# hanruihua/RDA-planner

Hardware: AMD Instinct MI355X
Metric: MPC steps/sec (ADMM early stop or iter_num cap: see residuals), T=20, N_obs=200 (higher is better)
Workload: dtype f64; 1 GPU; north-star: acker rectangle robot, T=20, N_obs=200 static seeded polygons, E=4, iter_num=4, iter_threshold=0.2, ro1=200; parallelism=single GPU

## Files before the change

rda_planner_amd/csrc/lammuz_device.h:

```cpp
#pragma once
#include <hip/hip_runtime.h>
#include <math.h>

#pragma clang fp contract(on)

namespace lmz {

constexpr int EMAX = 8;
constexpr int RMAX = 8;
constexpr double SIGN_TOL = 1e-12;

struct WaveLDS {
    double A[EMAX][2];
    double b[EMAX];
    double q[EMAX];
    double M[EMAX][2];
    unsigned char lamc[40];
    double vtx[28][2];
    int npv, nlv;
};
struct RobotLDS {
    double G[RMAX][2];
    double h[RMAX];
    unsigned char muc[40]; int nmv;
// ... 370 lines not shown
            Sol s;
            if (eval_candidate(W, Rb, P, il, im, ic, s)) {
                s.id = 2 * (il * nm + im) + ic;
                if (s.cost < best.cost || (s.cost == best.cost && s.id < best.id)) best = s;
            }
            mark(1 + 2 * ic + (itn < 1 ? itn : 1)); ++itn;
        }
        double bc = best.cost; int bid = best.id;
#pragma unroll
        for (int off = 32; off >= 1; off >>= 1) {
            double oc = __shfl_xor(bc, off, 64); int oid = __shfl_xor(bid, off, 64);
            if (oc < bc || (oc == bc && oid < bid)) { bc = oc; bid = oid; }
        }
        unsigned long long win = __ballot(best.id == bid);
        int src = __ffsll((long long)win) - 1;
        best.cost = __shfl(best.cost, src, 64); best.id = bid;
        best.m = __shfl(best.m, src, 64); best.H0 = __shfl(best.H0, src, 64); best.H1 = __shfl(best.H1, src, 64);
        best.i1 = __shfl(best.i1, src, 64); best.i2 = __shfl(best.i2, src, 64);
        best.j1 = __shfl(best.j1, src, 64); best.j2 = __shfl(best.j2, src, 64);
        best.l1 = __shfl(best.l1, src, 64); best.l2 = __shfl(best.l2, src, 64);
        best.g1 = __shfl(best.g1, src, 64); best.g2 = __shfl(best.g2, src, 64);
        mark(5 + ic);
        if (best.m >= 0) break;
        if (ic == 0) best.cost += 0.5 * best.m * best.m;
    }
}

template <int CTRL> __device__ __forceinline__ double dpp_mov_f64(double v)
{
    int lo = __builtin_amdgcn_update_dpp(0, __double2loint(v), CTRL, 0xf, 0xf, false);
    int hi = __builtin_amdgcn_update_dpp(0, __double2hiint(v), CTRL, 0xf, 0xf, false);
    return __hiloint2double(hi, lo);
}
__device__ __forceinline__ double wave_max(double v)
{
    double o;
    o = dpp_mov_f64<0xB1>(v); v = o > v ? o : v;
    o = dpp_mov_f64<0x4E>(v); v = o > v ? o : v;
    o = dpp_mov_f64<0x141>(v); v = o > v ? o : v;
    o = dpp_mov_f64<0x140>(v); v = o > v ? o : v;
    o = __shfl_xor(v, 16, 64); v = o > v ? o : v;
    o = __shfl_xor(v, 32, 64); v = o > v ? o : v;
    return v;
}

__device__ __forceinline__ double row_max(double v)
{
    double o;
    o = dpp_mov_f64<0xB1>(v); v = o > v ? o : v;
    o = dpp_mov_f64<0x4E>(v); v = o > v ? o : v;
    o = dpp_mov_f64<0x141>(v); v = o > v ? o : v;
    o = dpp_mov_f64<0x140>(v); v = o > v ? o : v;
    return v;
}
template <int GW> struct Grp {
    static __device__ __forceinline__ unsigned long long ballot(bool p, int lane)
    {
        const unsigned long long b = __ballot(p);
        if (GW == 64) return b;
        return (b >> (lane & 48)) & 0xffffull;
    }
    static __device__ __forceinline__ double max(double v) { return GW == 64 ? wave_max(v) : row_max(v); }
    template <typename Tv> static __device__ __forceinline__ Tv bcast(Tv v, int src) { return __shfl(v, src, GW); }
};

__device__ __forceinline__ int support_neighbour(int c, int n, const unsigned char *cand, int ncand, int k)
// ... 150 lines not shown
        const unsigned long long okb = Grp<GW>::ballot(ok, wlane);
        int src = -1;
        if ((okb & 1) && m0 >= 0) src = 0; else if ((okb & 2) && m1 < 0) src = 1;
        if (src >= 0) {
            take(s, src, 2 * (il * nm0 + im) + src);
            if (certify()) return true;
        }
    }
    if (GW >= 16) {
        const int q = (lane >> 1) & 7, c = lane & 1;
        int nil = -1, nim = -1;
        if (lane < 16) {
            if (q < 4) { nil = support_neighbour(il, E, W.lamc, W.nlv, q); nim = im; }
            else { nil = il; nim = support_neighbour(im, R, Rb.muc, Rb.nmv, q - 4); }
        }
        bool ok = false;
        if (lane < 16 && nil >= 0 && nim >= 0) ok = eval_candidate(W, Rb, P, nil, nim, c, s);
        const bool valid = ok && (c == 0 ? s.m >= 0 : s.m < 0);
        const unsigned long long vb = Grp<GW>::ballot(valid, wlane);
        const bool use = valid && !(c == 1 && ((vb >> (lane - 1)) & 1ull));
        const double cost = use ? s.cost : INFINITY;
        const double cmin = -Grp<GW>::max(-cost);
        if (cmin < INFINITY) {
            const unsigned long long wb = Grp<GW>::ballot(use && cost == cmin, wlane);
            const int src = __ffsll((long long)wb) - 1;
            const int cid = Grp<GW>::bcast(2 * (nil * nm0 + nim) + c, src);
            take(s, src, cid);
            if (certify()) return true;
        }
    }
    return false;
}

template <int GW> __device__ __forceinline__ bool central_normal_wave(const WaveLDS &W, const RobotLDS &Rb, const Params &P, int wlane, Sol &best)
{
    const int lane = wlane & (GW - 1);
    if (!(best.m > 0) || !(best.H0 * best.H0 + best.H1 * best.H1 < 1e-8)) return false;
    double as0 = 0, as1 = 0;
    if (P.norm2) { if (best.i1 >= 0) { as0 = best.l1; as1 = best.l2; } }
    else {
        if (best.i1 >= 0) { as0 += best.l1 * W.A[best.i1][0]; as1 += best.l1 * W.A[best.i1][1]; }
        if (best.i2 >= 0) { as0 += best.l2 * W.A[best.i2][0]; as1 += best.l2 * W.A[best.i2][1]; }
    }
    if (!(as0 * as0 + as1 * as1 >= 1.0 - 1e-9)) return false;
    const int nv = P.norm2 ? 1 : W.npv, nr = Rb.nrv;
    if (nr < 3 || (!P.norm2 && nv < 3) || nv * nr > 64 || nv > GW || nr > GW) return false;
    const double off = P.norm2 ? W.b[2] : 0.0;
    const double ins = rsqrt(as0 * as0 + as1 * as1), u0 = as0 * ins, u1 = as1 * ins;
    bool fail = false; double thi = INFINITY, tlo = INFINITY;
    for (int pi = lane; pi < nv * nr; pi += GW) {
        const int k = pi / nr, j = pi - k * nr;
        const double vx = P.norm2 ? W.b[0] : W.vtx[k][0], vy = P.norm2 ? W.b[1] : W.vtx[k][1];
        const double rx = Rb.rv[j][0], ry = Rb.rv[j][1];
        const double wx = P.px - vx + (P.cs * rx - P.sn * ry), wy = P.py - vy + (P.sn * rx + P.cs * ry);
        const double cj = P.xi0 * rx + P.xi1 * ry + P.kappa0 + off;
        const double n2 = wx * wx + wy * wy;
        if (!(n2 > 0)) fail = fail || cj < 0;
        else {
            const double inw = rsqrt(n2), q = -cj * inw, hx = wx * inw, hy = wy * inw;
            if (q >= 1.0) fail = true;
            else if (q > -1.0) {
                if (u0 * hx + u1 * hy < q - 1e-15) fail = true;
                else {
                    const double sb = sqrt((1.0 - q) * (1.0 + q));
                    const double epx = q * hx - sb * hy, epy = sb * hx + q * hy;
                    const double emx = q * hx + sb * hy, emy = -sb * hx + q * hy;
                    const double cp = u0 * epx + u1 * epy, sp = u0 * epy - u1 * epx;
                    const double cm = u0 * emx + u1 * emy, sm = emx * u1 - emy * u0;
                    double th = INFINITY, tl = INFINITY;
                    if (sp >= 0 && cp > -1.0) th = sp / (1.0 + cp);
                    else if (sp < 0 && sp > -1e-15) th = 0.0;
                    if (sm >= 0 && cm > -1.0) tl = sm / (1.0 + cm);
                    else if (sm < 0 && sm > -1e-15) tl = 0.0;
                    if (th < thi) thi = th;
                    if (tl < tlo) tlo = tl;
                }
            }
        }
    }
    if (Grp<GW>::ballot(fail, wlane)) return false;
    thi = -Grp<GW>::max(-thi); tlo = -Grp<GW>::max(-tlo);
    if (isinf(thi) && isinf(tlo)) return false;
    double chh, shh, chl, shl;
    if (isinf(thi)) { chh = 0; shh = 1; } else { const double r = rsqrt(1.0 + thi * thi); chh = r; shh = thi * r; }
    if (isinf(tlo)) { chl = 0; shl = 1; } else { const double r = rsqrt(1.0 + tlo * tlo); chl = r; shl = tlo * r; }
    const double Cr = chh * chl + shh * shl, Sr = shh * chl - chh * shl;
    const double a0 = u0 * Cr - u1 * Sr, a1 = u1 * Cr + u0 * Sr;
    int i1 = -1, i2 = -1; double l1 = 0, l2 = 0;
    if (P.norm2) { i1 = 0; i2 = 1; l1 = a0; l2 = a1; }
    else {
        const double val = lane < nv ? a0 * W.vtx[lane < nv ? lane : 0][0] + a1 * W.vtx[lane < nv ? lane : 0][1] : -INFINITY, mx = Grp<GW>::max(val);
        const int kb = __ffsll((long long)Grp<GW>::ballot(val == mx, wlane)) - 1;
        decode_pair((int)W.lamc[kb] - 1 - P.E, P.E, i1, i2);
        const double a00 = W.A[i1][0], a01 = W.A[i1][1], a10 = W.A[i2][0], a11 = W.A[i2][1], det = a00 * a11 - a01 * a10;
        l1 = (a0 * a11 - a10 * a1) / det;
        l2 = (a00 * a1 - a0 * a01) / det;
        if (l1 < -1e-9 || l2 < -1e-9) return false;
        if (l1 < 0) l1 = 0;
        if (l2 < 0) l2 = 0;
    }
    const double gx = -(P.cs * a0 + P.sn * a1) - P.xi0, gy = -(-P.sn * a0 + P.cs * a1) - P.xi1;
    int j1, j2; double g1, g2;
    {
        const double val = lane < nr ? gx * Rb.rv[lane < nr ? lane : 0][0] + gy * Rb.rv[lane < nr ? lane : 0][1] : -INFINITY, mx = Grp<GW>::max(val);
        const int jb = __ffsll((long long)Grp<GW>::ballot(val == mx, wlane)) - 1;
        decode_pair((int)Rb.muc[jb] - 1 - P.R, P.R, j1, j2);
        const double a00 = Rb.G[j1][0], a01 = Rb.G[j1][1], a10 = Rb.G[j2][0], a11 = Rb.G[j2][1], det = a00 * a11 - a01 * a10;
        g1 = (gx * a11 - a10 * gy) / det;
        g2 = (a00 * gy - gx * a01) / det;
        if (g1 < -1e-9 || g2 < -1e-9) return false;
        if (g1 < 0) g1 = 0;
        if (g2 < 0) g2 = 0;
    }
    double m = P.kappa0 - g1 * Rb.h[j1] - g2 * Rb.h[j2];
    double H0 = P.xi0 + g1 * Rb.G[j1][0] + g2 * Rb.G[j2][0], H1 = P.xi1 + g1 * Rb.G[j1][1] + g2 * Rb.G[j2][1];
    if (P.norm2) {
        m += l1 * W.q[0] + l2 * W.q[1] - W.q[2];
        H0 += l1 * W.M[0][0] + l2 * W.M[1][0] - W.M[2][0]; H1 += l1 * W.M[0][1] + l2 * W.M[1][1] - W.M[2][1];
    } else {
        m += l1 * W.q[i1] + l2 * W.q[i2];
        H0 += l1 * W.M[i1][0] + l2 * W.M[i2][0]; H1 += l1 * W.M[i1][1] + l2 * W.M[i2][1];
    }
    if (m < 0) return false;
    best.i1 = i1; best.i2 = i2; best.l1 = l1; best.l2 = l2; best.j1 = j1; best.j2 = j2; best.g1 = g1; best.g2 = g2;
    best.m = m; best.H0 = H0; best.H1 = H1;
    return true;
}

__device__ __forceinline__ double lam_of(const Sol &s, int norm2, int e)
{
    if (norm2) {
        if (s.i1 < 0) return 0.0;
        return e == 0 ? s.l1 : (e == 1 ? s.l2 : (e == 2 ? -hypot(s.l1, s.l2) : 0.0));
    }
    return e == s.i1 ? s.l1 : (e == s.i2 ? s.l2 : 0.0);
}
__device__ __forceinline__ double mu_of(const Sol &s, int j) { return j == s.j1 ? s.g1 : (j == s.j2 ? s.g2 : 0.0); }

}

#pragma clang fp contract(fast)
```

rda_planner_amd/csrc/rda_hip.hip:

```cpp
#include <hip/hip_runtime.h>
#include <climits>
#include <cstdio>
#include <cstdlib>
#include <cstring>
#include <vector>
#include <chrono>
#include <memory>
#include <dlfcn.h>
#include "../../include/rda_hip.h"
#include "host_buf.h"
#include "lammuz_device.h"
#include "lammuz_cp_device.h"
#include "lammuz_ip_device.h"
#include "su_device.h"
#include "scene_device.h"
#include "lidar_device.h"
#include "track_device.h"
#include "rollout_device.h"

#define HIPCHK(x) do { hipError_t e_ = (x); if (e_ != hipSuccess) { \
    fprintf(stderr, "librda_hip: %s failed: %s (%s:%d)\n", #x, hipGetErrorString(e_), __FILE__, __LINE__); return RDA_ERR_HIP; } } while (0)

struct Ctrl {
    int stop, iters, su_status, ipm_iters, st_tmp, it_tmp;
// ... 367 lines not shown
    return o;
}

__device__ __forceinline__ void block_partial(const Dev &d, int t, int j, const double (*rowv)[6], int q)
{
    const size_t bi = (size_t)t * d.J + j;
    if (q < NBS) {
        double acc = 0;
        for (int r = 0; r < GS; ++r) acc += rowv[r][q];
        __hip_atomic_store(bsum_arr(d, d.rank) + bi * NBS + q, acc, __ATOMIC_RELAXED, __HIP_MEMORY_SCOPE_AGENT);
    } else if (q == NBS) {
        unsigned long long m = 0;
        for (int r = 0; r < GS; ++r) m |= rowv[r][5] != 0.0 ? 1ull << r : 0ull;
        __hip_atomic_store(bmask_arr(d, d.rank) + bi, m, __ATOMIC_RELAXED, __HIP_MEMORY_SCOPE_AGENT);
    }
}
__device__ __forceinline__ void row_record(double *rv, const Dev &d, const RowOut &o, double px, double py)
{
    const su::RowTerm q = su::row_term(o.ax, o.ay, o.c4, o.c5, o.bl + o.c3, px, py, d.c.max_sd, true);
    rv[0] = q.aa; rv[1] = q.ga; rv[2] = q.gxa; rv[3] = o.res; rv[4] = o.hh; rv[5] = (!d.c.accelerated || q.near) ? 1.0 : 0.0;
}

__device__ __forceinline__ size_t hint_key(const Dev &d, int n, int t)
{
    int key = n;
    if (d.slot_src && n < d.src_used) { const int src = d.slot_src[n]; if (src >= 0 && src < d.src_cap) key = d.c.N + src; }
    return (size_t)t * d.hint_stride + key;
}
__device__ __forceinline__ int hint_read(const Dev &d, int par, int n, int t, bool first)
{
    return d.hint[(size_t)(par ^ 1) * d.hint_len + hint_key(d, n, first && t + 1 < d.c.T ? t + 1 : t)];
}
__device__ __forceinline__ void hint_write(const Dev &d, int par, int n, int t, int v) { d.hint[(size_t)par * d.hint_len + hint_key(d, n, t)] = v; }

__device__ __forceinline__ void lammuz_body(const Dev &d, const int block, const int it)
{
#pragma clang fp contract(on)
    __shared__ lmz::WaveLDS wl[4];
    __shared__ lmz::RobotLDS rb;
    const int T = d.c.T, N = d.c.N, E = d.c.E, R = d.c.R;
    if (d.ctrl->stop) return;
    const int lane = threadIdx.x & 63, wv = threadIdx.x >> 6;
    if (d.obstacle_num == 0) {
        if (block == 0 && d.rank == (N - 1) / d.Nloc)
            for (int t = threadIdx.x; t < T; t += 256) {
                int i = t * d.Nloc + (N - 1) % d.Nloc;
                coef_arr(d, d.rank, 0)[i] = 0; coef_arr(d, d.rank, 1)[i] = 0; coef_arr(d, d.rank, 2)[i] = 0;
                coef_arr(d, d.rank, 8)[i] = coef_arr(d, d.rank, 3)[i];
            }
        return;
    }
    if (threadIdx.x < 2 * R) rb.G[threadIdx.x >> 1][threadIdx.x & 1] = d.G[threadIdx.x];
    if (threadIdx.x >= 64 && threadIdx.x < 64 + R) rb.h[threadIdx.x - 64] = d.h[threadIdx.x - 64];
    if (threadIdx.x >= 128 && threadIdx.x < 128 + 40) rb.muc[threadIdx.x - 128] = d.muc[threadIdx.x - 128];
    if (threadIdx.x >= 192 && threadIdx.x < 192 + 56) (&rb.rv[0][0])[threadIdx.x - 192] = (&d.rv[0][0])[threadIdx.x - 192];
    if (threadIdx.x == 255) { rb.nmv = d.nmv; rb.nrv = d.nrv; }
    const int w = block * 4 + wv;
    int t, nl; unit_of(d, w, t, nl);
    const bool live = t < T && nl < d.Nlive;
    if (!live) { t = 0; nl = 0; }
    const int n = d.rank * d.Nloc + nl;
    lmz::WaveLDS &W = wl[wv];
    const size_t ao = ((size_t)n * d.nt + (d.nt > 1 ? t + 1 : 0)) * E;
    if (lane < 2 * E) W.A[lane >> 1][lane & 1] = d.A[ao * 2 + lane];
    if (lane < E) W.b[lane] = d.b[ao + lane];
    __syncthreads();
// ... 53 lines not shown
        res = (v - prev) * (v - prev); d.mu[o * R + j] = v;
    } else if (lane == E + R) {
        double old = d.z[zi];
        res = (znew - old) * (znew - old); d.z[zi] = znew;
    }
#pragma unroll
    for (int off = 32; off >= 1; off >>= 1) res += __shfl_xor(res, off, 64);
    if (lane == 0) {
        double ax = 0, ay = 0, bl = 0, mh = 0, gx = 0, gy = 0;
        for (int i = 0; i < E; ++i) {
            double v = lmz::lam_of(best, P.norm2, i);
            ax += v * W.A[i][0]; ay += v * W.A[i][1]; bl += v * W.b[i];
        }
        for (int j = 0; j < R; ++j) {
            double v = lmz::mu_of(best, j);
            mh += v * rb.h[j]; gx += v * rb.G[j][0]; gy += v * rb.G[j][1];
        }
        const double hx = gx + P.cs * ax + P.sn * ay, hy = gy - P.sn * ax + P.cs * ay;
        const double xin0 = P.xi0 + hx, xin1 = P.xi1 + hy;
        d.xi[2 * o] = xin0; d.xi[2 * o + 1] = xin1;
        const double im = ax * P.px + ay * P.py - bl - mh;
        const double zetan = zeta + im - dbar - znew;
        d.zeta[zi] = zetan;
        RowOut ro; ro.ax = ax; ro.ay = ay; ro.bl = bl; ro.c3 = mh + znew - zetan; ro.c4 = gx + xin0; ro.c5 = gy + xin1;
        ro.res = res; ro.hh = hx * hx + hy * hy;
        store_row(d, k, ro);
    }
}

__global__ __launch_bounds__(256) void k_lammuz(Dev d, int it) { lammuz_body(d, blockIdx.x, it); }

#ifdef RDA_LMZ_CLK
__device__ unsigned long long *g_lmz_clk = nullptr;
__device__ int *g_lmz_faillog = nullptr;
#endif
template <int MODE = 0, bool CW = false> __device__ __forceinline__ void lammuz_body_rows(const Dev &d, const int block, const int nblocks, const int it, const Fin &fin)
{
#pragma clang fp contract(on)
    constexpr int WPB = GS / 4;
    __shared__ lmz::WaveLDS wl[GS];
    __shared__ lmz::RobotLDS rb;
    __shared__ double rowv[MODE == 0 ? GS : 1][6];
    const int T = d.c.T, E = d.c.E, R = d.c.R;
#ifdef RDA_LMZ_CLK
    long long clk_prev = clock64(); const long long clk_in = clk_prev; bool clk_enum = false; const unsigned long long clk_wall_in = (unsigned long long)wall_clock64();
    unsigned long long *const clk_slot = g_lmz_clk ? g_lmz_clk + 16 * (size_t)(block * (GS / 4) + (threadIdx.x >> 6)) : nullptr;
#define LMZ_CLK(k) do { if (MODE == 0) { const long long now_ = clock64(); if (clk_slot && (threadIdx.x & 63) == 0) clk_slot[k] += (unsigned long long)(now_ - clk_prev); clk_prev = now_; } } while (0)
#else
#define LMZ_CLK(k) do { } while (0)
#endif
    int tb = 0, jb = 0;
    if (MODE != 2) { block_of(d, block, tb, jb); if (tb < 0) return; }
    const int lane = threadIdx.x & 63, wv = threadIdx.x >> 6, row = lane >> 4, gl = lane & 15;
    struct Early { double px, py, cs, sn, xi0, xi1, zeta, dbar, prev, vtx[4], A, b, G, h, zold; int cone, src, hpar, hint, npv, nlv; unsigned char lamc[3]; } ey;
    if (MODE == 0) {
        const int nl0 = jb * GS + wv * 4 + row, nl = nl0 < d.Nlive ? nl0 : 0, n = d.rank * d.Nloc + nl;
        ey.src = (d.slot_src && n < d.src_used) ? d.slot_src[n] : -1;
        ey.hpar = d.ctrl->hint_par & 1;
    }
    if (d.ctrl->stop) return;
    if (MODE == 2 && block * WPB >= d.ctrl->wl_count + (d.ctrl->wlc_count + 3) / 4) return;
    LMZ_CLK(0);
    if (MODE == 0) {
        const int t = tb, nl0 = jb * GS + wv * 4 + row, nl = nl0 < d.Nlive ? nl0 : 0, n = d.rank * d.Nloc + nl;
        const double *ps = d.pose + 4 * t;
        const size_t o = drow(d, n, t + 1), zi = drow(d, n, t), oc = (size_t)n * d.nt + (d.nt > 1 ? t + 1 : 0);
        ey.px = ps[0]; ey.py = ps[1]; ey.cs = ps[2]; ey.sn = ps[3];
        ey.xi0 = d.xi[2 * o]; ey.xi1 = d.xi[2 * o + 1]; ey.zeta = d.zeta[zi]; ey.dbar = d.dis[t]; ey.cone = d.cone[n];
        ey.zold = d.z[zi];
        ey.prev = *(gl < E ? &d.lam[o * E + gl] : (gl < E + R ? &d.mu[o * R + gl - E] : &d.lam[o * E]));
        {
            const size_t ao = ((size_t)n * d.nt + (d.nt > 1 ? t + 1 : 0)) * E;
            ey.A = d.A[ao * 2 + (gl < 2 * E ? gl : 0)]; ey.b = d.b[ao + (gl < E ? gl : 0)];
            ey.G = d.G[(int)threadIdx.x < 2 * R ? threadIdx.x : 0]; ey.h = d.h[(int)threadIdx.x < R ? threadIdx.x : 0];
        }
#pragma unroll
        for (int k = 0; k < 3; ++k) ey.lamc[k] = gl + 16 * k < d.oc_ls ? d.oc_lamc[oc * d.oc_ls + gl + 16 * k] : (unsigned char)0;
#pragma unroll
        for (int k = 0; k < 4; ++k) ey.vtx[k] = gl + 16 * k < d.oc_vs ? d.oc_vtx[oc * d.oc_vs + gl + 16 * k] : 0.0;
        ey.npv = d.oc_cnt[2 * oc]; ey.nlv = d.oc_cnt[2 * oc + 1];
        {
            const int key = (ey.src >= 0 && ey.src < d.src_cap) ? d.c.N + ey.src : n, tr = (it == 0 && t + 1 < T) ? t + 1 : t;
            ey.hint = d.hint[(size_t)(ey.hpar ^ 1) * d.hint_len + (size_t)tr * d.hint_stride + key];
        }
    }
    if (MODE == 0) {
        if ((int)threadIdx.x < 2 * R) rb.G[threadIdx.x >> 1][threadIdx.x & 1] = ey.G;
        if ((int)threadIdx.x < R) rb.h[threadIdx.x] = ey.h;
    } else {
        for (int i = threadIdx.x; i < 2 * R; i += 64 * WPB) rb.G[i >> 1][i & 1] = d.G[i];
        for (int i = threadIdx.x; i < R; i += 64 * WPB) rb.h[i] = d.h[i];
    }
    for (int i = threadIdx.x; i < 40; i += 64 * WPB) rb.muc[i] = d.muc[i];
    for (int i = threadIdx.x; i < 56; i += 64 * WPB) (&rb.rv[0][0])[i] = (&d.rv[0][0])[i];
    if (threadIdx.x == 0) { rb.nmv = d.nmv; rb.nrv = d.nrv; }
    const int cntP = MODE == 2 ? d.ctrl->wl_count : 1, cntC = MODE == 2 ? d.ctrl->wlc_count : 0;
    const int cnt = cntP + (cntC + 3) / 4;
    for (int base = MODE == 2 ? block * WPB : 0; base < cnt; base += MODE == 2 ? nblocks * WPB : 1) {
    if (MODE == 2) __syncthreads();
    const bool entry = MODE == 2 && base + wv < cnt;
    int t, nl;
    bool live2 = false;
    if (MODE == 2) {
        const int sl = entry ? base + wv : base;
        int widx;
        if (sl < cntP) { widx = sl; live2 = entry && row == 0; }
        else { const int c0 = 4 * (sl - cntP), ci = c0 + row; live2 = entry && ci < cntC; widx = d.wl_cap - 1 - (live2 ? ci : c0); }
        unit_of(d, d.wl[widx], t, nl);
    } else { t = tb; nl = jb * GS + wv * 4 + row; }
    const bool live = MODE == 2 ? live2 : nl < d.Nlive;
    if (!live) nl = 0;
    const int n = d.rank * d.Nloc + nl;
    lmz::WaveLDS &W = wl[wv * 4 + row];
    const size_t ao = ((size_t)n * d.nt + (d.nt > 1 ? t + 1 : 0)) * E;
    if (MODE == 0) {
        if (gl < 2 * E) W.A[gl >> 1][gl & 1] = ey.A;
        if (gl < E) W.b[gl] = ey.b;
    } else {
        if (gl < 2 * E) W.A[gl >> 1][gl & 1] = d.A[ao * 2 + gl];
        if (gl < E) W.b[gl] = d.b[ao + gl];
    }
    __syncthreads();
    LMZ_CLK(1);
    lmz::Params P;
    P.E = E; P.R = R; P.norm2 = MODE == 0 ? ey.cone : d.cone[n];
    const double *ps = d.pose + 4 * t;
    if (MODE == 0) { P.px = ey.px; P.py = ey.py; P.cs = ey.cs; P.sn = ey.sn; }
    else { P.px = ps[0]; P.py = ps[1]; P.cs = ps[2]; P.sn = ps[3]; }
    const size_t o = drow(d, n, t + 1), zi = drow(d, n, t);
    if (MODE == 0) { P.xi0 = ey.xi0; P.xi1 = ey.xi1; } else { P.xi0 = d.xi[2 * o]; P.xi1 = d.xi[2 * o + 1]; }
    const double zeta = MODE == 0 ? ey.zeta : d.zeta[zi], dbar = MODE == 0 ? ey.dbar : d.dis[t];
    P.kappa0 = zeta - dbar; P.ro2 = d.c.ro2; P.delta = d.c.delta;
    lmz::Sol best;
    double prev = 0.0;
    if (MODE == 0) prev = gl < E + R ? ey.prev : 0.0;
    else if (gl < E) prev = d.lam[o * E + gl];
    else if (gl < E + R) prev = d.mu[o * R + gl - E];
    const double px0 = P.px, py0 = P.py;
    bool bad = !isfinite(P.px + P.py + P.cs + P.sn + P.xi0 + P.xi1 + P.kappa0);
    if (gl < 2 * E) bad = bad || !isfinite(W.A[gl >> 1][gl & 1]);
    if (gl < E) bad = bad || !isfinite(W.b[gl]);
    bad = ((__ballot(bad) >> (16 * row)) & 0xffffull) != 0;
    if (bad) {
        if (gl < 2 * E) W.A[gl >> 1][gl & 1] = 0;
        if (gl < E) W.b[gl] = 0;
        P.px = P.py = P.sn = P.xi0 = P.xi1 = P.kappa0 = 0; P.cs = 1;
    }
    lmz::wave_sync();
    lmz::pose_products(W, P, gl);
    {
        const size_t oc = (size_t)n * d.nt + (d.nt > 1 ? t + 1 : 0);
        if (MODE == 0) {
#pragma unroll
            for (int k = 0; k < 3; ++k) if (gl + 16 * k < d.oc_ls) W.lamc[gl + 16 * k] = ey.lamc[k];
// ... 63 lines not shown
            const int rid = flist[i];
            lmz::Params Pg;
            { const Prm &q = prm[rid]; Pg.E = E; Pg.R = R; Pg.norm2 = q.norm2; Pg.px = q.px; Pg.py = q.py; Pg.cs = q.cs; Pg.sn = q.sn; Pg.xi0 = q.xi0; Pg.xi1 = q.xi1;
              Pg.kappa0 = q.kappa0; Pg.ro2 = P.ro2; Pg.delta = P.delta; }
            lmz::Sol bg;
            lmz::solve_wave(wl[rid], rb, Pg, lane, bg);
            if (lane == 0) sol[rid] = bg;
        }
        __syncthreads();
        if (mine) best = sol[wv * 4 + row];
        need = 0;
#ifdef RDA_LMZ_CLK
        clk_enum = nf > 0;
        if (mine && gl == 0 && live && g_lmz_faillog) {
            const int k = atomicAdd(&g_lmz_faillog[0], 1);
            if (k < 200000) { g_lmz_faillog[1 + 3 * k] = hint_in; g_lmz_faillog[2 + 3 * k] = best.id >> 1; g_lmz_faillog[3 + 3 * k] = P.norm2; }
        }
#endif
    }
    LMZ_CLK(4);
    while (need) {
        const int g = (__ffsll((long long)need) - 1) >> 4;
        need &= ~(0xffffull << (16 * g));
        lmz::Params Pg;
        const int src = 16 * g;
        Pg.E = E; Pg.R = R; Pg.norm2 = __shfl(P.norm2, src, 64);
        Pg.px = __shfl(P.px, src, 64); Pg.py = __shfl(P.py, src, 64); Pg.cs = __shfl(P.cs, src, 64); Pg.sn = __shfl(P.sn, src, 64);
        Pg.xi0 = __shfl(P.xi0, src, 64); Pg.xi1 = __shfl(P.xi1, src, 64); Pg.kappa0 = __shfl(P.kappa0, src, 64);
        Pg.ro2 = P.ro2; Pg.delta = P.delta;
        lmz::Sol bg;
        lmz::solve_wave(wl[wv * 4 + g], rb, Pg, lane, bg);
        if (row == g) best = bg;
    }
    if (gl == 0 && live && !defer) hint_write(d, hpar, n, t, best.id >> 1);
    if (d.centre) lmz::central_normal_wave<16>(W, rb, P, lane, best);
    LMZ_CLK(5);
    bad = bad || !(isfinite(best.cost) && isfinite(best.m) && isfinite(best.H0) && isfinite(best.H1));
    const double znew = (d.c.accelerated ? 0.5 : 1.0) * (best.m > 0 ? best.m : 0.0);
    double res = 0;
    const bool wr = live && !bad && !defer;
    if (gl < E) {
        double v = lmz::lam_of(best, P.norm2, gl);
        res = (v - prev) * (v - prev); if (wr) d.lam[o * E + gl] = v;
    } else if (gl < E + R) {
        int j = gl - E;
        double v = lmz::mu_of(best, j);
        res = (v - prev) * (v - prev); if (wr) d.mu[o * R + j] = v;
    } else if (gl == E + R) {
        const double old = MODE == 0 ? ey.zold : d.z[zi];
        res = (znew - old) * (znew - old); if (wr) d.z[zi] = znew;
    }
#pragma unroll
    for (int off = 8; off >= 1; off >>= 1) res += __shfl_xor(res, off, 16);
    if (gl == 0) {
        const int k = t * d.Nloc + nl;
        RowOut ro;
        bool have = false;
        if (live && bad) {
            ro = failed_row(d, k); have = true;
            store_row(d, k, ro);
            hint_write(d, hpar, n, t, -1);
            atomicAdd(&d.ctrl->lmz_fail, 1);
        } else if (wr) {
            double ax = 0, ay = 0, bl = 0, mh = 0, gx = 0, gy = 0;
            for (int i = 0; i < E; ++i) {
                double v = lmz::lam_of(best, P.norm2, i);
                ax += v * W.A[i][0]; ay += v * W.A[i][1]; bl += v * W.b[i];
            }
            for (int j = 0; j < R; ++j) {
                double v = lmz::mu_of(best, j);
                mh += v * rb.h[j]; gx += v * rb.G[j][0]; gy += v * rb.G[j][1];
            }
            const double hx = gx + P.cs * ax + P.sn * ay, hy = gy - P.sn * ax + P.cs * ay;
            const double xin0 = P.xi0 + hx, xin1 = P.xi1 + hy;
            d.xi[2 * o] = xin0; d.xi[2 * o + 1] = xin1;
            const double im = ax * P.px + ay * P.py - bl - mh;
            const double zetan = zeta + im - dbar - znew;
            d.zeta[zi] = zetan;
            ro.ax = ax; ro.ay = ay; ro.bl = bl; ro.c3 = mh + znew - zetan; ro.c4 = gx + xin0; ro.c5 = gy + xin1;
            ro.res = res; ro.hh = hx * hx + hy * hy; have = true;
            store_row(d, k, ro);
        }
        if (MODE == 0) {
            double *rv = rowv[wv * 4 + row];
            if (have) row_record(rv, d, ro, px0, py0);
            else { rv[0] = rv[1] = rv[2] = rv[3] = rv[4] = rv[5] = 0.0; }
        }
    }
    LMZ_CLK(6);
    if (MODE == 0) {
        __syncthreads();
        block_partial(d, tb, jb, rowv, threadIdx.x);
        if (block == 0 && threadIdx.x == 0) d.ctrl->pose_ok = 1;
    }
    LMZ_CLK(7);
#ifdef RDA_LMZ_CLK
    if (MODE == 0 && clk_slot && (threadIdx.x & 63) == 0) {
        const unsigned long long tot = (unsigned long long)(clock64() - clk_in);
        clk_slot[8] += 1; clk_slot[9] += tot; if (tot > clk_slot[10]) clk_slot[10] = tot;
        clk_slot[13] = clk_wall_in; clk_slot[14] = (unsigned long long)wall_clock64();
        if (clk_enum) { clk_slot[11] += 1; clk_slot[12] += tot; }
    }
#endif
    }
#undef LMZ_CLK
}

__global__ __launch_bounds__(64 * GS / 4) void k_lammuz_rows(Dev d, int it, Fin fin) { warm_kernargs<sizeof(Dev) + sizeof(int) + sizeof(Fin)>(); lammuz_body_rows<0, true>(d, blockIdx.x, gridDim.x, it, fin); }
__global__ __launch_bounds__(64 * GS / 4, 2) void k_lammuz_rows_dense(Dev d, int it, Fin fin) { lammuz_body_rows<0>(d, blockIdx.x, gridDim.x, it, fin); }
__global__ __launch_bounds__(64 * GS / 4, 3) void k_lammuz_rows_fast(Dev d, int it) { lammuz_body_rows<1>(d, blockIdx.x, gridDim.x, it, Fin{}); }
__global__ __launch_bounds__(64 * GS / 4, 1) void k_lammuz_enum(Dev d, int it) { lammuz_body_rows<2>(d, blockIdx.x, gridDim.x, it, Fin{}); }

constexpr int FPB = 256 / GS;
__device__ __forceinline__ void finalize_body(const Dev &d, const int block, const int nblocks, const int it, const Fin &fin)
{
#pragma clang fp contract(on)
    __shared__ double rowv[FPB][GS][6];
    if (it >= 0 && d.ctrl->stop) return;
    const int T = d.c.T, g = threadIdx.x / GS, row = threadIdx.x % GS;
    const int B = block * FPB + g, t = B / d.J, j = B - t * d.J, nl = GS * j + row;
    double *rv = rowv[g][row];
    if (B < T * d.J && nl < d.Nlive) {
        const int k = t * d.Nloc + nl;
        RowOut ro; ro.ax = coef_arr(d, d.rank, 0)[k]; ro.ay = coef_arr(d, d.rank, 1)[k]; ro.bl = coef_arr(d, d.rank, 2)[k];
        ro.c3 = coef_arr(d, d.rank, 3)[k]; ro.c4 = coef_arr(d, d.rank, 4)[k]; ro.c5 = coef_arr(d, d.rank, 5)[k];
        ro.res = coef_arr(d, d.rank, 6)[k]; ro.hh = coef_arr(d, d.rank, 7)[k];
        row_record(rv, d, ro, d.pose[4 * t], d.pose[4 * t + 1]);
    } else { rv[0] = rv[1] = rv[2] = rv[3] = rv[4] = rv[5] = 0.0; }
    __syncthreads();
    if (B < T * d.J) block_partial(d, t, j, rowv[g], row);
    if (block == 0 && threadIdx.x == 0) d.ctrl->pose_ok = 1;
}
__global__ __launch_bounds__(256) void k_lmz_finalize(Dev d, int it, Fin fin) { finalize_body(d, blockIdx.x, gridDim.x, it, fin); }

template <int NX, int MX> __device__ __forceinline__ void lammuz_cp_body(const Dev &d, const int block)
{
    const int T = d.c.T, E = d.c.E, R = d.c.R;
    if (d.ctrl->stop) return;
// ... 1388 lines not shown
    TraceSet t;
    if (t.alloc((size_t)K, ns, nu)) return RDA_ERR_HIP;
    HIPCHK(hipMemcpy(t.s, nom_s, K * ns * sizeof(double), hipMemcpyHostToDevice));
    HIPCHK(hipMemcpy(t.u, nom_u, K * nu * sizeof(double), hipMemcpyHostToDevice));
    HIPCHK(hipMemcpy(t.ref, ref_s, K * ns * sizeof(double), hipMemcpyHostToDevice));
    HIPCHK(hipMemcpy(t.speed, ref_speed, K * sizeof(double), hipMemcpyHostToDevice));
    H->trace = std::move(t);
    return RDA_OK;
}

extern "C" int rda_enqueue_step(rda_handle *H, int k)
{
    if (!H || k < 0 || k >= H->trace.K) return RDA_ERR_ARG;
    const size_t ns = traj_s(H->d.c.T), nu = traj_u(H->d.c.T);
    return enqueue_admm(H, H->trace.s + k * ns, H->trace.u + k * nu, H->trace.ref + k * ns, H->trace.speed + k,
                        H->trace.out_u + k * nu, H->trace.out_s + k * ns, H->trace.info + k);
}

extern "C" int rda_enqueue_range(rda_handle *H, int k0, int k1)
{
    if (!H || k0 < 0 || k1 > H->trace.K || k0 > k1) return RDA_ERR_ARG;
    for (int k = k0; k < k1; ++k) { int rc = rda_enqueue_step(H, k); if (rc != RDA_OK) return rc; }
    return RDA_OK;
}

#ifdef RDA_LMZ_CLK
extern "C" int rda_debug_lmz_clk(rda_handle *H, unsigned long long *out, int max_waves)
{
    static unsigned long long *buf = nullptr; static int cap = 0;
    static hbuf::Group &keep = *new hbuf::Group;
    HIPCHK(hipStreamSynchronize(H->stream));
    if (!buf) {
        hbuf::Group g; unsigned long long *b;
        if (g.dev(&b, (size_t)max_waves * 16)) return RDA_ERR_HIP;
        HIPCHK(hipMemcpyToSymbol(HIP_SYMBOL(g_lmz_clk), &b, sizeof(b)));
        keep.d.push_back(std::move(g.d[0])); buf = b; cap = max_waves;
        return RDA_OK;
    }
    if (max_waves < 0) {
        static int *flog = nullptr;
        if (!flog) {
            hbuf::Group g; int *f;
            if (g.dev(&f, 1 + 3 * 200000)) return RDA_ERR_HIP;
            HIPCHK(hipMemcpyToSymbol(HIP_SYMBOL(g_lmz_faillog), &f, sizeof(f)));
            keep.d.push_back(std::move(g.d[0])); flog = f;
            return RDA_OK;
        }
        HIPCHK(hipMemcpy(out, flog, (1 + 3 * 200000) * sizeof(int), hipMemcpyDeviceToHost));
        HIPCHK(hipMemset(flog, 0, sizeof(int)));
        return RDA_OK;
    }
    if (max_waves > cap) return RDA_ERR_ARG;
    HIPCHK(hipMemcpy(out, buf, (size_t)max_waves * 16 * sizeof(unsigned long long), hipMemcpyDeviceToHost));
    HIPCHK(hipMemset(buf, 0, (size_t)cap * 16 * sizeof(unsigned long long)));
    return RDA_OK;
}
#endif
#ifdef RDA_LMZ_STATS
extern "C" int rda_debug_lmz_stats(rda_handle *H, unsigned *out)
{
    HIPCHK(hipStreamSynchronize(H->stream));
    HIPCHK(hipMemcpy(out, (char *)H->d.ctrl + offsetof(Ctrl, lmz_stat), 8 * sizeof(unsigned), hipMemcpyDeviceToHost));
    return RDA_OK;
}
#endif
extern "C" int rda_sync(rda_handle *H) { if (!H) return RDA_ERR_ARG; HIPCHK(hipStreamSynchronize(H->stream)); H->tick.pending_scene = 0; return RDA_OK; }

extern "C" int rda_fetch_result(rda_handle *H, int k, double *out_u, double *out_s, rda_info *info)
{
    if (!H || k < 0 || k >= H->trace.K) return RDA_ERR_ARG;
    const size_t ns = traj_s(H->d.c.T), nu = traj_u(H->d.c.T);
    HIPCHK(hipStreamSynchronize(H->stream));
    if (out_u) HIPCHK(hipMemcpy(out_u, H->trace.out_u + k * nu, nu * sizeof(double), hipMemcpyDeviceToHost));
    if (out_s) HIPCHK(hipMemcpy(out_s, H->trace.out_s + k * ns, ns * sizeof(double), hipMemcpyDeviceToHost));
    if (info) HIPCHK(hipMemcpy(info, H->trace.info + k, sizeof(rda_info), hipMemcpyDeviceToHost));
    return RDA_OK;
}

extern "C" int rda_timing_reset(rda_handle *H, int enable)
{
    if (!H) return RDA_ERR_ARG;
    HIPCHK(hipStreamSynchronize(H->stream));
    HIPCHK(hipStreamSynchronize(H->stream2));
    H->timing = enable; H->ev_used[0] = H->ev_used[1] = H->ev_used[2] = H->ev_used[3] = 0;
    return RDA_OK;
}
extern "C" int rda_timing_read(rda_handle *H, int which, double *total_ms, int *launches)
// ... 1850 lines not shown
```

Baseline: 4205 steps/s.

## Spread lammuz row epilogue across lanes and trim scalar work in the wide kernel

In the CW (k_lammuz_rows) path, the robot tables are loaded early per thread, and the stop flag and hint parity become wave-uniform via readfirstlane. The central normal routine uses branchless selects. The lam/mu/z residual writes become lane-parallel, and the 16-lane residual reduction uses DPP row moves instead of shuffles. The per-row A/G dot products, once serial loops on lane 0, become a DPP shift-accumulate across lanes. Hint writes now key on the source slot. Extra clock sub-markers are added for profiling. The aim is to cut serial lane-0 work and shuffle latency in the epilogue, at the cost of more complex lane logic and a changed hint key.

```diff
diff --git a/rda_planner_amd/csrc/lammuz_device.h b/rda_planner_amd/csrc/lammuz_device.h
--- a/rda_planner_amd/csrc/lammuz_device.h
+++ b/rda_planner_amd/csrc/lammuz_device.h
@@ -426,6 +426,12 @@
     int hi = __builtin_amdgcn_update_dpp(0, __double2hiint(v), CTRL, 0xf, 0xf, false);
     return __hiloint2double(hi, lo);
 }
+template <int CTRL> __device__ __forceinline__ double dpp_mov0_f64(double v)
+{
+    int lo = __builtin_amdgcn_update_dpp(0, __double2loint(v), CTRL, 0xf, 0xf, true);
+    int hi = __builtin_amdgcn_update_dpp(0, __double2hiint(v), CTRL, 0xf, 0xf, true);
+    return __hiloint2double(hi, lo);
+}
 __device__ __forceinline__ double wave_max(double v)
 {
     double o;
@@ -642,7 +648,12 @@
     return false;
 }
 
-template <int GW> __device__ __forceinline__ bool central_normal_wave(const WaveLDS &W, const RobotLDS &Rb, const Params &P, int wlane, Sol &best)
+#ifdef RDA_LMZ_CLK
+#define LMZ_CN_MARK(k) do { if (clk) clk[k] = clock64(); } while (0)
+#else
+#define LMZ_CN_MARK(k) do { } while (0)
+#endif
+template <int GW, bool SIDE = false> __device__ __forceinline__ bool central_normal_wave(const WaveLDS &W, const RobotLDS &Rb, const Params &P, int wlane, Sol &best, long long *clk = nullptr)
 {
     const int lane = wlane & (GW - 1);
     if (!(best.m > 0) || !(best.H0 * best.H0 + best.H1 * best.H1 < 1e-8)) return false;
@@ -658,6 +669,7 @@
     const double off = P.norm2 ? W.b[2] : 0.0;
     const double ins = rsqrt(as0 * as0 + as1 * as1), u0 = as0 * ins, u1 = as1 * ins;
     bool fail = false; double thi = INFINITY, tlo = INFINITY;
+    LMZ_CN_MARK(0);
     for (int pi = lane; pi < nv * nr; pi += GW) {
         const int k = pi / nr, j = pi - k * nr;
         const double vx = P.norm2 ? W.b[0] : W.vtx[k][0], vy = P.norm2 ? W.b[1] : W.vtx[k][1];
@@ -678,24 +690,39 @@
                     const double cp = u0 * epx + u1 * epy, sp = u0 * epy - u1 * epx;
                     const double cm = u0 * emx + u1 * emy, sm = emx * u1 - emy * u0;
                     double th = INFINITY, tl = INFINITY;
+                    if (SIDE) {
+                        const double qh = sp / (1.0 + cp), ql = sm / (1.0 + cm);
+                        th = (sp >= 0 && cp > -1.0) ? qh : ((sp < 0 && sp > -1e-15) ? 0.0 : INFINITY);
+                        tl = (sm >= 0 && cm > -1.0) ? ql : ((sm < 0 && sm > -1e-15) ? 0.0 : INFINITY);
+                    } else {
                     if (sp >= 0 && cp > -1.0) th = sp / (1.0 + cp);
                     else if (sp < 0 && sp > -1e-15) th = 0.0;
                     if (sm >= 0 && cm > -1.0) tl = sm / (1.0 + cm);
                     else if (sm < 0 && sm > -1e-15) tl = 0.0;
+                    }
                     if (th < thi) thi = th;
                     if (tl < tlo) tlo = tl;
                 }
             }
         }
     }
+    LMZ_CN_MARK(1);
     if (Grp<GW>::ballot(fail, wlane)) return false;
     thi = -Grp<GW>::max(-thi); tlo = -Grp<GW>::max(-tlo);
     if (isinf(thi) && isinf(tlo)) return false;
     double chh, shh, chl, shl;
+    if (SIDE) {
+        const double rh = rsqrt(1.0 + thi * thi), rl = rsqrt(1.0 + tlo * tlo);
+        const double sh = thi * rh, sl = tlo * rl;
+        const bool ih = isinf(thi), il = isinf(tlo);
+        chh = ih ? 0.0 : rh; shh = ih ? 1.0 : sh; chl = il ? 0.0 : rl; shl = il ? 1.0 : sl;
+    } else {
     if (isinf(thi)) { chh = 0; shh = 1; } else { const double r = rsqrt(1.0 + thi * thi); chh = r; shh = thi * r; }
     if (isinf(tlo)) { chl = 0; shl = 1; } else { const double r = rsqrt(1.0 + tlo * tlo); chl = r; shl = tlo * r; }
+    }
     const double Cr = chh * chl + shh * shl, Sr = shh * chl - chh * shl;
     const double a0 = u0 * Cr - u1 * Sr, a1 = u1 * Cr + u0 * Sr;
+    LMZ_CN_MARK(2);
     int i1 = -1, i2 = -1; double l1 = 0, l2 = 0;
     if (P.norm2) { i1 = 0; i2 = 1; l1 = a0; l2 = a1; }
     else {
@@ -709,6 +736,7 @@
         if (l1 < 0) l1 = 0;
         if (l2 < 0) l2 = 0;
     }
+    LMZ_CN_MARK(3);
     const double gx = -(P.cs * a0 + P.sn * a1) - P.xi0, gy = -(-P.sn * a0 + P.cs * a1) - P.xi1;
     int j1, j2; double g1, g2;
     {
@@ -722,6 +750,7 @@
         if (g1 < 0) g1 = 0;
         if (g2 < 0) g2 = 0;
     }
+    LMZ_CN_MARK(4);
     double m = P.kappa0 - g1 * Rb.h[j1] - g2 * Rb.h[j2];
     double H0 = P.xi0 + g1 * Rb.G[j1][0] + g2 * Rb.G[j2][0], H1 = P.xi1 + g1 * Rb.G[j1][1] + g2 * Rb.G[j2][1];
     if (P.norm2) {
@@ -747,6 +776,8 @@
 }
 __device__ __forceinline__ double mu_of(const Sol &s, int j) { return j == s.j1 ? s.g1 : (j == s.j2 ? s.g2 : 0.0); }
 
+#undef LMZ_CN_MARK
+
 }
 
 #pragma clang fp contract(fast)
diff --git a/rda_planner_amd/csrc/rda_hip.hip b/rda_planner_amd/csrc/rda_hip.hip
--- a/rda_planner_amd/csrc/rda_hip.hip
+++ b/rda_planner_amd/csrc/rda_hip.hip
@@ -423,6 +423,11 @@
     return d.hint[(size_t)(par ^ 1) * d.hint_len + hint_key(d, n, first && t + 1 < d.c.T ? t + 1 : t)];
 }
 __device__ __forceinline__ void hint_write(const Dev &d, int par, int n, int t, int v) { d.hint[(size_t)par * d.hint_len + hint_key(d, n, t)] = v; }
+__device__ __forceinline__ void hint_write_src(const Dev &d, int par, int n, int t, int src, int v)
+{
+    const int key = (src >= 0 && src < d.src_cap) ? d.c.N + src : n;
+    d.hint[(size_t)par * d.hint_len + (size_t)t * d.hint_stride + key] = v;
+}
 
 __device__ __forceinline__ void lammuz_body(const Dev &d, const int block, const int it)
 {
@@ -542,32 +547,45 @@
 
 #ifdef RDA_LMZ_CLK
 __device__ unsigned long long *g_lmz_clk = nullptr;
+constexpr int LMZ_CLK_WORDS = 32;
 __device__ int *g_lmz_faillog = nullptr;
 #endif
 template <int MODE = 0, bool CW = false> __device__ __forceinline__ void lammuz_body_rows(const Dev &d, const int block, const int nblocks, const int it, const Fin &fin)
 {
 #pragma clang fp contract(on)
     constexpr int WPB = GS / 4;
+    constexpr bool LANES = CW;
     __shared__ lmz::WaveLDS wl[GS];
     __shared__ lmz::RobotLDS rb;
     __shared__ double rowv[MODE == 0 ? GS : 1][6];
     const int T = d.c.T, E = d.c.E, R = d.c.R;
 #ifdef RDA_LMZ_CLK
     long long clk_prev = clock64(); const long long clk_in = clk_prev; bool clk_enum = false; const unsigned long long clk_wall_in = (unsigned long long)wall_clock64();
-    unsigned long long *const clk_slot = g_lmz_clk ? g_lmz_clk + 16 * (size_t)(block * (GS / 4) + (threadIdx.x >> 6)) : nullptr;
-#define LMZ_CLK(k) do { if (MODE == 0) { const long long now_ = clock64(); if (clk_slot && (threadIdx.x & 63) == 0) clk_slot[k] += (unsigned long long)(now_ - clk_prev); clk_prev = now_; } } while (0)
+    unsigned long long *const clk_slot = g_lmz_clk ? g_lmz_clk + LMZ_CLK_WORDS * (size_t)(block * (GS / 4) + (threadIdx.x >> 6)) : nullptr;
+    long long clk_sub = clk_prev;
+#define LMZ_CLK(k) do { if (MODE == 0) { const long long now_ = clock64(); if (clk_slot && (threadIdx.x & 63) == 0) clk_slot[k] += (unsigned long long)(now_ - clk_prev); clk_prev = now_; clk_sub = now_; } } while (0)
+#define LMZ_SUB(k) do { if (MODE == 0) { const long long now_ = clock64(); if (clk_slot && (threadIdx.x & 63) == 0) clk_slot[16 + (k)] += (unsigned long long)(now_ - clk_sub); clk_sub = now_; } } while (0)
 #else
 #define LMZ_CLK(k) do { } while (0)
+#define LMZ_SUB(k) do { } while (0)
 #endif
     int tb = 0, jb = 0;
     if (MODE != 2) { block_of(d, block, tb, jb); if (tb < 0) return; }
     const int lane = threadIdx.x & 63, wv = threadIdx.x >> 6, row = lane >> 4, gl = lane & 15;
-    struct Early { double px, py, cs, sn, xi0, xi1, zeta, dbar, prev, vtx[4], A, b, G, h, zold; int cone, src, hpar, hint, npv, nlv; unsigned char lamc[3]; } ey;
+    struct Early { double px, py, cs, sn, xi0, xi1, zeta, dbar, prev, vtx[4], A, b, G, h, zold, rv; int cone, src, hpar, hint, npv, nlv; unsigned char lamc[3], muc; } ey;
     if (MODE == 0) {
         const int nl0 = jb * GS + wv * 4 + row, nl = nl0 < d.Nlive ? nl0 : 0, n = d.rank * d.Nloc + nl;
         ey.src = (d.slot_src && n < d.src_used) ? d.slot_src[n] : -1;
         ey.hpar = d.ctrl->hint_par & 1;
-    }
+        static_assert(64 * WPB >= 56, "one element of the robot tables per thread");
+        if (LANES) { ey.muc = d.muc[(int)threadIdx.x < 40 ? threadIdx.x : 0]; ey.rv = (&d.rv[0][0])[(int)threadIdx.x < 56 ? threadIdx.x : 0]; }
+    }
+    if (LANES) {
+        int stop = d.ctrl->stop;
+        asm volatile("" : "+v"(ey.hpar), "+v"(stop));
+        ey.hpar = __builtin_amdgcn_readfirstlane(ey.hpar);
+        if (__builtin_amdgcn_readfirstlane(stop)) return;
+    } else
     if (d.ctrl->stop) return;
     if (MODE == 2 && block * WPB >= d.ctrl->wl_count + (d.ctrl->wlc_count + 3) / 4) return;
     LMZ_CLK(0);
@@ -594,6 +612,7 @@
             ey.hint = d.hint[(size_t)(ey.hpar ^ 1) * d.hint_len + (size_t)tr * d.hint_stride + key];
         }
     }
+    LMZ_SUB(0);
     if (MODE == 0) {
         if ((int)threadIdx.x < 2 * R) rb.G[threadIdx.x >> 1][threadIdx.x & 1] = ey.G;
         if ((int)threadIdx.x < R) rb.h[threadIdx.x] = ey.h;
@@ -601,9 +620,15 @@
         for (int i = threadIdx.x; i < 2 * R; i += 64 * WPB) rb.G[i >> 1][i & 1] = d.G[i];
         for (int i = threadIdx.x; i < R; i += 64 * WPB) rb.h[i] = d.h[i];
     }
-    for (int i = threadIdx.x; i < 40; i += 64 * WPB) rb.muc[i] = d.muc[i];
-    for (int i = threadIdx.x; i < 56; i += 64 * WPB) (&rb.rv[0][0])[i] = (&d.rv[0][0])[i];
+    if (LANES) {
+        if ((int)threadIdx.x < 40) rb.muc[threadIdx.x] = ey.muc;
+        if ((int)threadIdx.x < 56) (&rb.rv[0][0])[threadIdx.x] = ey.rv;
+    } else {
+        for (int i = threadIdx.x; i < 40; i += 64 * WPB) rb.muc[i] = d.muc[i];
+        for (int i = threadIdx.x; i < 56; i += 64 * WPB) (&rb.rv[0][0])[i] = (&d.rv[0][0])[i];
+    }
     if (threadIdx.x == 0) { rb.nmv = d.nmv; rb.nrv = d.nrv; }
+    LMZ_SUB(1);
     const int cntP = MODE == 2 ? d.ctrl->wl_count : 1, cntC = MODE == 2 ? d.ctrl->wlc_count : 0;
     const int cnt = cntP + (cntC + 3) / 4;
     for (int base = MODE == 2 ? block * WPB : 0; base < cnt; base += MODE == 2 ? nblocks * WPB : 1) {
@@ -630,6 +655,7 @@
         if (gl < 2 * E) W.A[gl >> 1][gl & 1] = d.A[ao * 2 + gl];
         if (gl < E) W.b[gl] = d.b[ao + gl];
     }
+    LMZ_SUB(2);
     __syncthreads();
     LMZ_CLK(1);
     lmz::Params P;
@@ -759,13 +785,32 @@
         lmz::solve_wave(wl[wv * 4 + g], rb, Pg, lane, bg);
         if (row == g) best = bg;
     }
-    if (gl == 0 && live && !defer) hint_write(d, hpar, n, t, best.id >> 1);
-    if (d.centre) lmz::central_normal_wave<16>(W, rb, P, lane, best);
+    if (gl == 0 && live && !defer) {
+        if (LANES) hint_write_src(d, hpar, n, t, ey.src, best.id >> 1); else hint_write(d, hpar, n, t, best.id >> 1);
+    }
+    LMZ_SUB(3);
+#ifdef RDA_LMZ_CLK
+    {
+        long long cn[5]; for (int q = 0; q < 5; ++q) cn[q] = 0;
+        if (d.centre) lmz::central_normal_wave<16, LANES>(W, rb, P, lane, best, cn);
+        if (MODE == 0 && clk_slot && (threadIdx.x & 63) == 0) { long long pv = clk_sub; for (int q = 0; q < 5; ++q) if (cn[q]) { clk_slot[20 + q] += (unsigned long long)(cn[q] - pv); pv = cn[q]; } }
+    }
+#else
+    if (d.centre) lmz::central_normal_wave<16, LANES>(W, rb, P, lane, best);
+#endif
     LMZ_CLK(5);
     bad = bad || !(isfinite(best.cost) && isfinite(best.m) && isfinite(best.H0) && isfinite(best.H1));
     const double znew = (d.c.accelerated ? 0.5 : 1.0) * (best.m > 0 ? best.m : 0.0);
     double res = 0;
     const bool wr = live && !bad && !defer;
+    if (LANES) {
+        const bool isl = gl < E, ism = !isl && gl < E + R, isz = gl == E + R;
+        const double vlam = lmz::lam_of(best, P.norm2, gl), vmu = lmz::mu_of(best, gl - E);
+        const double v = isl ? vlam : (ism ? vmu : znew), old = isz ? ey.zold : prev;
+        res = (isl || ism || isz) ? (v - old) * (v - old) : 0.0;
+        double *const p = isl ? &d.lam[o * E + gl] : (ism ? &d.mu[o * R + gl - E] : &d.z[zi]);
+        if (wr && gl <= E + R) *p = v;
+    } else
     if (gl < E) {
         double v = lmz::lam_of(best, P.norm2, gl);
         res = (v - prev) * (v - prev); if (wr) d.lam[o * E + gl] = v;
@@ -777,8 +822,31 @@
         const double old = MODE == 0 ? ey.zold : d.z[zi];
         res = (znew - old) * (znew - old); if (wr) d.z[zi] = znew;
     }
+    LMZ_SUB(9);
+    if (LANES) {
+        res += lmz::dpp_mov0_f64<0x128>(res);
+        res += lmz::dpp_mov0_f64<0x124>(res);
+        res += lmz::dpp_mov0_f64<0x4E>(res);
+        res += lmz::dpp_mov0_f64<0xB1>(res);
+    } else {
 #pragma unroll
-    for (int off = 8; off >= 1; off >>= 1) res += __shfl_xor(res, off, 16);
+        for (int off = 8; off >= 1; off >>= 1) res += __shfl_xor(res, off, 16);
+    }
+    LMZ_SUB(10);
+    double ax = 0, ay = 0, bl = 0, mh = 0, gx = 0, gy = 0;
+    if (LANES) {
+        const bool le = gl < E, lr = gl < R;
+        const int ie = le ? E - 1 - gl : 0, je = lr ? R - 1 - gl : 0;
+        const double a0r = W.A[ie][0], a1r = W.A[ie][1], bbr = W.b[ie], hhr = rb.h[je], g0r = rb.G[je][0], g1r = rb.G[je][1];
+        const double vl = le ? lmz::lam_of(best, P.norm2, ie) : 0.0, vm = lr ? lmz::mu_of(best, je) : 0.0;
+        const double a0 = le ? a0r : 0.0, a1 = le ? a1r : 0.0, bb = le ? bbr : 0.0, hh = lr ? hhr : 0.0, g0 = lr ? g0r : 0.0, g1 = lr ? g1r : 0.0;
+        const int ns = E > R ? E : R;
+        for (int s = 0; s < ns; ++s) {
+            ax = vl * a0 + lmz::dpp_mov0_f64<0x101>(ax); ay = vl * a1 + lmz::dpp_mov0_f64<0x101>(ay); bl = vl * bb + lmz::dpp_mov0_f64<0x101>(bl);
+            mh = vm * hh + lmz::dpp_mov0_f64<0x101>(mh); gx = vm * g0 + lmz::dpp_mov0_f64<0x101>(gx); gy = vm * g1 + lmz::dpp_mov0_f64<0x101>(gy);
+        }
+        LMZ_SUB(11);
+    }
     if (gl == 0) {
         const int k = t * d.Nloc + nl;
         RowOut ro;
@@ -786,17 +854,19 @@
         if (live && bad) {
             ro = failed_row(d, k); have = true;
             store_row(d, k, ro);
-            hint_write(d, hpar, n, t, -1);
+            if (LANES) hint_write_src(d, hpar, n, t, ey.src, -1); else hint_write(d, hpar, n, t, -1);
             atomicAdd(&d.ctrl->lmz_fail, 1);
         } else if (wr) {
-            double ax = 0, ay = 0, bl = 0, mh = 0, gx = 0, gy = 0;
-            for (int i = 0; i < E; ++i) {
-                double v = lmz::lam_of(best, P.norm2, i);
-                ax += v * W.A[i][0]; ay += v * W.A[i][1]; bl += v * W.b[i];
-            }
-            for (int j = 0; j < R; ++j) {
-                double v = lmz::mu_of(best, j);
-                mh += v * rb.h[j]; gx += v * rb.G[j][0]; gy += v * rb.G[j][1];
+            if (!LANES) {
+                for (int i = 0; i < E; ++i) {
+                    double v = lmz::lam_of(best, P.norm2, i);
+                    ax += v * W.A[i][0]; ay += v * W.A[i][1]; bl += v * W.b[i];
+                }
+                for (int j = 0; j < R; ++j) {
+                    double v = lmz::mu_of(best, j);
+                    mh += v * rb.h[j]; gx += v * rb.G[j][0]; gy += v * rb.G[j][1];
+                }
+                LMZ_SUB(11);
             }
             const double hx = gx + P.cs * ax + P.sn * ay, hy = gy - P.sn * ax + P.cs * ay;
             const double xin0 = P.xi0 + hx, xin1 = P.xi1 + hy;
@@ -807,6 +877,7 @@
             ro.ax = ax; ro.ay = ay; ro.bl = bl; ro.c3 = mh + znew - zetan; ro.c4 = gx + xin0; ro.c5 = gy + xin1;
             ro.res = res; ro.hh = hx * hx + hy * hy; have = true;
             store_row(d, k, ro);
+            LMZ_SUB(12);
         }
         if (MODE == 0) {
             double *rv = rowv[wv * 4 + row];
@@ -817,6 +888,7 @@
     LMZ_CLK(6);
     if (MODE == 0) {
         __syncthreads();
+        LMZ_SUB(13);
         block_partial(d, tb, jb, rowv, threadIdx.x);
         if (block == 0 && threadIdx.x == 0) d.ctrl->pose_ok = 1;
     }
@@ -831,6 +903,7 @@
 #endif
     }
 #undef LMZ_CLK
+#undef LMZ_SUB
 }
 
 __global__ __launch_bounds__(64 * GS / 4) void k_lammuz_rows(Dev d, int it, Fin fin) { warm_kernargs<sizeof(Dev) + sizeof(int) + sizeof(Fin)>(); lammuz_body_rows<0, true>(d, blockIdx.x, gridDim.x, it, fin); }
@@ -2285,7 +2358,7 @@
     HIPCHK(hipStreamSynchronize(H->stream));
     if (!buf) {
         hbuf::Group g; unsigned long long *b;
-        if (g.dev(&b, (size_t)max_waves * 16)) return RDA_ERR_HIP;
+        if (g.dev(&b, (size_t)max_waves * LMZ_CLK_WORDS)) return RDA_ERR_HIP;
         HIPCHK(hipMemcpyToSymbol(HIP_SYMBOL(g_lmz_clk), &b, sizeof(b)));
         keep.d.push_back(std::move(g.d[0])); buf = b; cap = max_waves;
         return RDA_OK;
@@ -2304,8 +2377,8 @@
         return RDA_OK;
     }
     if (max_waves > cap) return RDA_ERR_ARG;
-    HIPCHK(hipMemcpy(out, buf, (size_t)max_waves * 16 * sizeof(unsigned long long), hipMemcpyDeviceToHost));
-    HIPCHK(hipMemset(buf, 0, (size_t)cap * 16 * sizeof(unsigned long long)));
+    HIPCHK(hipMemcpy(out, buf, (size_t)max_waves * LMZ_CLK_WORDS * sizeof(unsigned long long), hipMemcpyDeviceToHost));
+    HIPCHK(hipMemset(buf, 0, (size_t)cap * LMZ_CLK_WORDS * sizeof(unsigned long long)));
     return RDA_OK;
 }
 #endif
```

After: 4283 steps/s, median of 6. 1.02x the previous value.
